# ben-hayes/neural-waveshaping-synthesis

Measured on AMD Instinct MI355X. Metric: audio_samples_per_sec, higher is better.
Workload: dtype f32 (fp16x2-split MFMA contractions = 22-bit products, fp32 accumulate; FiLM interpolation bf16x3-split MFMA = exact fp32 operands); 1 GPU; NEWT forward, vn checkpoint, FastNEWT LUT, batch 64/GPU x 500 frames (4 s @ 16 kHz), torch.rand F0/control, RNG draws on device; batch_per_gpu=64, frames=500, samples_per_utterance=64000, parallelism=batch-shard x1, exciter_opts=0, streams=2

## Files before the change

neural-waveshaping-synthesis_amd/build.py:

```python
import concurrent.futures as cf
import hashlib
import os
import subprocess
import sys

HERE = os.path.dirname(os.path.abspath(__file__))
CSRC = os.path.join(HERE, "csrc")
OBJ = os.path.join(HERE, "csrc", "_obj")
LIB = os.path.join(HERE, "libnws_hip.so")
OPS_LIB = os.path.join(HERE, "libnws_torch_ops.so")
PROBE_LIB = os.path.join(HERE, "libnws_probe.so")
SOURCES = ["exciter_newt.hip", "control_gru.hip", "frame_mlps.hip", "fir_noise.hip", "reverb_fft.hip", "forward.hip",
           "loudness.hip", "stages.hip", "generic.hip", "stream.hip", "queue_probe.hip", "exchange.hip"]
PROBE_SOURCES = ["coexec_probe.hip"]
FLAGS = ["--offload-arch=gfx950", "-O3", "-std=c++17", "-ffp-contract=off", "-fPIC", "-fvisibility=default",
         "-Wall", "-Wno-unused-function", "-Wno-pass-failed", "-Rpass-analysis=kernel-resource-usage"]
KEEP_SLP = ("fir_noise.hip", "control_gru.hip")
EXTRA_FLAGS = {src: ["-fno-slp-vectorize"] for src in SOURCES + PROBE_SOURCES if src not in KEEP_SLP}
FLAGS += [f for f in os.environ.get("NWS_EXTRA_HIPCC_FLAGS", "").split() if f]
LLVM_BIN = "/opt/rocm/lib/llvm/bin"
SWIZZLE_ALLOW = ("pk_probe_kernel", "pk_probe2_kernel", "pk_probe_mixed_kernel")


def _hipcc():
    for c in (os.environ.get("HIPCC"), "/opt/rocm/bin/hipcc", "hipcc"):
        if c and (os.path.isabs(c) and os.path.exists(c) or not os.path.isabs(c)):
            return c
    raise RuntimeError("hipcc not found")


def _stamp():
    h = hashlib.sha256((" ".join(FLAGS) + repr(sorted(EXTRA_FLAGS.items()))).encode())
    for f in sorted(os.listdir(CSRC)):
        p = os.path.join(CSRC, f)
        if os.path.isfile(p) and f != "torch_ops.cpp":
            h.update(f.encode())
            h.update(open(p, "rb").read())
    for hdr in ("nws_hip.h", "nws_hip_debug.h", "nws_probe.h"):
        h.update(open(os.path.join(HERE, "..", "include", hdr), "rb").read())
    return h.hexdigest()


def device_disassembly(obj):
    import tempfile
    with tempfile.TemporaryDirectory() as td:
        fat, co = os.path.join(td, "fat.bin"), os.path.join(td, "dev.co")
        r = subprocess.run([os.path.join(LLVM_BIN, "llvm-objcopy"), "--dump-section", f".hip_fatbin={fat}", obj,
                            os.path.join(td, "host.o")], capture_output=True, text=True)
        if r.returncode != 0:
            if "not found" in r.stderr:
                return ""
            raise RuntimeError(f"llvm-objcopy failed on {obj}: {r.stderr}")
        subprocess.run([os.path.join(LLVM_BIN, "clang-offload-bundler"), "--unbundle", "--type=o", f"--input={fat}",
                        "--targets=hipv4-amdgcn-amd-amdhsa--gfx950", f"--output={co}"], check=True, capture_output=True)
        return subprocess.run([os.path.join(LLVM_BIN, "llvm-objdump"), "-d", co], check=True, capture_output=True,
                              text=True).stdout


def check_packed_swizzles(obj, allow=None):
    import re
    allow = SWIZZLE_ALLOW if allow is None else allow
    found, kernel = [], None
    for line in device_disassembly(obj).splitlines():
        m = re.match(r"^[0-9a-f]+ <(\S+)>:", line)
        if m:
            kernel = m.group(1)
            continue
        m = re.search(r"\b(v_\w+)\b.*?op_sel:\[\d,(\d)", line)
        if m and m.group(2) == "1" and not any(a in (kernel or "") for a in allow):
            found.append((kernel, " ".join(line.split("//")[0].split())))
    return found


def _vgprs(tok):
    import re
    m = re.fullmatch(r"v\[(\d+):(\d+)\]", tok)
    if m:
        return set(range(int(m.group(1)), int(m.group(2)) + 1))
    m = re.fullmatch(r"v(\d+)", tok)
    return {int(m.group(1))} if m else set()


def check_valu_mfma_hazard(obj, wait_states=2):
    import re
    found, kernel, window = [], None, []
    for line in device_disassembly(obj).splitlines():
        m = re.match(r"^[0-9a-f]+ <(\S+)>:", line)
        if m:
            kernel, window = m.group(1), []
            continue
        parts = line.split("//")[0].split("\t")
        text = " ".join(" ".join(parts[1:]).split()) if len(parts) > 1 else ""
        if not text:
            continue
        op = text.split()[0]
        ops = [t.strip() for t in text[len(op):].split(",")]
        if op.startswith("v_mfma") or op.startswith("v_smfmac"):
            srcs = set().union(*[_vgprs(t.split()[0]) for t in ops[1:4] if t])
            left = wait_states
            for ws, dst, ptext in reversed(window):
                if left <= 0:
                    break
                if dst & srcs:
                    found.append((kernel, ptext, text))
                left -= ws
        if op == "s_nop":
            window.append((int(ops[0], 0) + 1, set(), text))
        elif op.startswith("s_cbranch") or op in ("s_branch", "s_barrier", "s_endpgm", "s_setpc_b64"):
            window = []
        elif op.startswith("v_") and not op.startswith("v_mfma") and not op.startswith("v_smfmac") and not op.startswith("v_cmp"):
            window.append((1, _vgprs(ops[0].split()[0]) if ops and ops[0] else set(), text))
        else:
            window.append((1, set(), text))
        window = window[-8:]
    return found


REGISTER_BUDGETS = (
    ("exciter_newt_kernelILi4ELi2ELi2E", 80, "default oscillator kernel: three 8-wave workgroups per CU"),
    ("exciter_newt_kernelILi4ELi2ELi6E", 80, "one-term variant: three 8-wave workgroups per CU"),
    ("exciter_newt_kernelILi4ELi2ELi10E", 80, "hybrid variant: three 8-wave workgroups per CU"),
    ("exciter_newt_kernelILi4ELi2ELi26E", 80, "hybrid-W variant: three 8-wave workgroups per CU"),
    ("exciter_newt_kernelILi5ELi1ELi0E", 128, "exact-shaper bank kernel: four 4-wave workgroups per CU (38.8 KB of LDS each)"),
    ("exciter_newt_kernelILi6ELi1ELi0E", 128, "exact-shaper bank kernel (no v_fract): four 4-wave workgroups per CU"),
    ("g_exciter_newt_mfma_kernel", 128, "runtime-size oscillator kernel: four 4-wave workgroups per CU"),
)


def kernel_registers(remarks):
    regs, name = {}, None
    for line in remarks.splitlines():
        if "Function Name:" in line:
            name = line.split("Function Name:")[1].split("[-Rpass")[0].strip()
            regs[name] = 0
        elif name is not None and (" VGPRs:" in line or " AGPRs:" in line) and "Spill" not in line:
            regs[name] += int(line.split("GPRs:")[1].split()[0])
    return regs


def check_register_budgets(remarks, budgets=None):
    over = []
    for kernel, n in kernel_registers(remarks).items():
        for key, budget, why in (REGISTER_BUDGETS if budgets is None else budgets):
            if key in kernel and n > budget:
                over.append((kernel, n, budget, why))
    return over


def build_torch_ops(force=False, verbose=True):
    try:
        import torch
        from torch.utils import cpp_extension as ce
    except Exception as e:
        print(f"torch not importable ({e}): skipping libnws_torch_ops.so", file=sys.stderr)
        return None
    src = os.path.join(CSRC, "torch_ops.cpp")
    h = hashlib.sha256(open(src, "rb").read())
    h.update(open(os.path.join(HERE, "..", "include", "nws_hip.h"), "rb").read())
    h.update(open(os.path.join(HERE, "..", "include", "nws_hip_debug.h"), "rb").read())
    h.update(torch.__version__.encode())
    stamp, stamp_file = h.hexdigest(), OPS_LIB + ".stamp"
    if not force and os.path.exists(OPS_LIB) and os.path.exists(stamp_file) and open(stamp_file).read() == stamp:
        return OPS_LIB
    tlib = os.path.join(os.path.dirname(torch.__file__), "lib")
    cmd = ["g++", "-O2", "-std=c++17", "-fPIC", "-shared", "-D__HIP_PLATFORM_AMD__", "-DUSE_ROCM",
           f"-D_GLIBCXX_USE_CXX11_ABI={int(torch._C._GLIBCXX_USE_CXX11_ABI)}", "-Wall", "-Wno-unused-function",
           *[f"-I{p}" for p in ce.include_paths()], "-I/opt/rocm/include", src, "-o", OPS_LIB,
           f"-L{HERE}", "-lnws_hip", f"-L{tlib}", "-ltorch", "-ltorch_cpu", "-lc10", "-lc10_hip", "-ltorch_hip",
           "-Wl,-rpath,$ORIGIN", f"-Wl,-rpath,{tlib}"]
    r = subprocess.run(cmd, capture_output=True, text=True)
    if r.returncode != 0:
        raise RuntimeError(f"g++ failed on torch_ops.cpp:\n{r.stderr[-6000:]}")
    with open(stamp_file, "w") as f:
        f.write(stamp)
    if verbose:
        print(f"built {OPS_LIB}")
    return OPS_LIB


def build(force=False, verbose=True):
    lib = build_hip(force, verbose)
    build_torch_ops(force, verbose)
    return lib


def build_hip(force=False, verbose=True):
    stamp_file = LIB + ".stamp"
    stamp = _stamp()
    if (not force and os.path.exists(LIB) and os.path.exists(PROBE_LIB) and os.path.exists(stamp_file)
            and open(stamp_file).read() == stamp):
        return LIB
    os.makedirs(OBJ, exist_ok=True)
    hipcc = _hipcc()

    def compile_one(src):
        obj = os.path.join(OBJ, src.replace(".hip", ".o"))
        cmd = [hipcc, *FLAGS, *EXTRA_FLAGS.get(src, []), "-c", os.path.join(CSRC, src), "-o", obj]
        r = subprocess.run(cmd, capture_output=True, text=True)
        if r.returncode != 0:
            raise RuntimeError(f"hipcc failed on {src}:\n{r.stderr}")
        name, spilled, rest, skip = None, [], [], 0
        for line in r.stderr.splitlines():
            if skip and (line.lstrip().startswith("|") or line.lstrip().split(" ")[0].isdigit()):
                skip -= 1
                continue
            skip = 0
            if "remark:" in line:
                skip = 2
                if "Function Name:" in line:
                    name = line.split("Function Name:")[1].split("[-Rpass")[0].strip()
                elif "ScratchSize [bytes/lane]:" in line and int(line.split("ScratchSize [bytes/lane]:")[1].split()[0]) != 0:
                    spilled.append(name)
            else:
                rest.append(line)
        if spilled:
            if os.environ.get("NWS_BUILD_ALLOW_SCRATCH") == "1":
                print(f"{src}: kernels using scratch memory (allowed by NWS_BUILD_ALLOW_SCRATCH): {spilled}", file=sys.stderr)
            else:
                raise RuntimeError(f"{src}: kernels using scratch memory (spills or stack): {spilled}")
        over = check_register_budgets(r.stderr)
        if over:
            lines = "\n".join(f"  {k}: {n} registers > {b} ({why})" for k, n, b, why in over)
            raise RuntimeError(f"{src}: kernels over their register budget (REGISTER_BUDGETS: workgroups per CU):\n{lines}")
        swz = check_packed_swizzles(obj, SWIZZLE_ALLOW if src in PROBE_SOURCES else ())
        if swz:
            lines = "\n".join(f"  {k}: {i}" for k, i in swz[:12])
            raise RuntimeError(f"{src}: packed fp32 instructions with a swizzled src1 low lane (co-execution hazard, see "
                               f"check_packed_swizzles):\n{lines}")
        haz = check_valu_mfma_hazard(obj)
        if haz:
            lines = "\n".join(f"  {k}: {p}  ->  {m}" for k, p, m in haz[:12])
            raise RuntimeError(f"{src}: v_mfma reads a VGPR that a VALU instruction wrote less than 2 wait states earlier (inline asm "
                               f"in front of a matrix instruction? see check_valu_mfma_hazard):\n{lines}")
        if verbose and "\n".join(rest).strip():
            print("\n".join(rest), file=sys.stderr)
        return obj

    with cf.ThreadPoolExecutor(max_workers=len(SOURCES) + len(PROBE_SOURCES)) as ex:
        objs = list(ex.map(compile_one, SOURCES + PROBE_SOURCES))
    for lib, these in ((LIB, objs[:len(SOURCES)]), (PROBE_LIB, objs[len(SOURCES):])):
        r = subprocess.run([hipcc, "--offload-arch=gfx950", "-shared", "-fPIC", *these, "-o", lib], capture_output=True, text=True)
        if r.returncode != 0:
            raise RuntimeError(f"link failed:\n{r.stderr}")
    with open(stamp_file, "w") as f:
        f.write(stamp)
    if verbose:
        print(f"built {LIB}")
    return LIB


if __name__ == "__main__":
    build(force="--force" in sys.argv)
```

neural-waveshaping-synthesis_amd/csrc/fir_noise.hip:

```cpp
#include <type_traits>

#include "nws_common.h"

namespace {

constexpr int kL = NWS_FIR_LEN;
constexpr int kHop = NWS_HOP;
constexpr int kHalf = NWS_FIR_HALF;
constexpr int kHopsPerBlock = 4;

struct NoiseLds {
  float taps[kHopsPerBlock + 1][kL];
  float taps1[kHopsPerBlock + 1][kL];
  float sig[(kHopsPerBlock + 1) * kHop + kHop];
};

__device__ __forceinline__ float padded_noise(const float* __restrict__ noise, int len, int origin, int i) {
  int s = i - origin;
  if (s < 0) s = -s;
  if (s > len - 1) s = 2 * (len - 1) - s;
  s = s < 0 ? 0 : s;
  return noise[s];
}

__device__ __forceinline__ float row_noise(const float* __restrict__ noise, int lo, int hi, int origin, int i) {
  int s = i - origin;
  if (s < lo) s = 2 * lo - s;
  if (s > hi) s = 2 * hi - s;
  s = s < 0 ? 0 : s;
  return noise[s];
}

template <bool ROWS>
__global__ __launch_bounds__(256) void fir_noise_kernel(const float* __restrict__ fir, const float* __restrict__ noise,
                                                        const float* __restrict__ add_in, int T, int len, int origin,
                                                        float* __restrict__ out, const int4* __restrict__ rows) {
  __shared__ __attribute__((aligned(16))) NoiseLds L;
  const int tid = threadIdx.x, lane = tid & 63, wave = tid >> 6;
  const int half = lane >> 5, q = lane & 31;
  const int b = blockIdx.y;
  const int t0 = blockIdx.x * kHopsPerBlock;
  const int N = T * kHop;
  int4 rb = make_int4(0, 0, 0, 0);
  if constexpr (ROWS) rb = rows[b];
  const int t_lo = ROWS ? rb.z : 0;

  for (int e = tid; e < (kHopsPerBlock + 1) * kL; e += 256) {
    const int fr = e >> 8, k = e & 255;
    const int t = t0 - 1 + fr;
    const int d = k >= kHalf ? k - kHalf : kHalf - k;
    const float v = (t >= t_lo && t < T && d < kHalf) ? fir[((size_t)b * T + t) * kHalf + d] : 0.0f;
    L.taps[fr][k] = v;
    L.taps1[fr][(k + 1) & 255] = v;
  }
  for (int e = tid; e < (kHopsPerBlock + 1) * kHop + kHop; e += 256) {
    const int i = (t0 - 1) * kHop + e;
    float v = 0.0f;
    if (i >= 0 && i < N + kL - 1) v = ROWS ? row_noise(noise, rb.x, rb.y, origin, i) : padded_noise(noise, len, origin, i);
    L.sig[e] = v;
  }
  __syncthreads();

  const int t = t0 + wave;
  if (t >= T) return;
  const int slot = wave + 1 - half;
  const int nb = half * kHop + 4 * q;
  const float* f = &L.sig[slot * kHop];
  const float* h = L.taps[slot];

  const float* h1 = L.taps1[slot];
  f32x2 a0 = {0.0f, 0.0f}, a1 = {0.0f, 0.0f}, a2 = {0.0f, 0.0f}, a3 = {0.0f, 0.0f};
  float4 hi0 = *reinterpret_cast<const float4*>(&h[nb & 255]);
  float4 hi1 = *reinterpret_cast<const float4*>(&h1[nb & 255]);
#pragma unroll 4
  for (int m0 = 0; m0 < kL; m0 += 4) {
    const float4 lo0 = *reinterpret_cast<const float4*>(&h[(nb - m0 - 4) & 255]);
    const float4 lo1 = *reinterpret_cast<const float4*>(&h1[(nb - m0 - 4) & 255]);
    const float4 fv = *reinterpret_cast<const float4*>(&f[m0]);
    const f32x2 fs0 = {fv.y, fv.x}, fs1 = {fv.w, fv.z};
    a1 = fma2(fs0, f32x2{hi0.x, hi0.y}, a1);
    a3 = fma2(fs0, f32x2{hi0.z, hi0.w}, a3);
    a1 = fma2(fs1, f32x2{lo0.z, lo0.w}, a1);
    a3 = fma2(fs1, f32x2{hi0.x, hi0.y}, a3);
    a0 = fma2(fs0, f32x2{hi1.x, hi1.y}, a0);
    a2 = fma2(fs0, f32x2{hi1.z, hi1.w}, a2);
    a0 = fma2(fs1, f32x2{lo1.z, lo1.w}, a0);
    a2 = fma2(fs1, f32x2{hi1.x, hi1.y}, a2);
    hi0 = lo0;
    hi1 = lo1;
  }
  const float y0 = a0.x + a0.y, y1 = a1.x + a1.y, y2 = a2.x + a2.y, y3 = a3.x + a3.y;
  const float o0 = y0 + nws_swap_halves(y0);
  const float o1 = y1 + nws_swap_halves(y1);
  const float o2 = y2 + nws_swap_halves(y2);
  const float o3 = y3 + nws_swap_halves(y3);
  if (half == 0) {
    const float inv = t == t_lo ? 1.0f : 0.5f;
    const size_t o = (size_t)b * N + (size_t)t * kHop + 4 * q;
    float4 r = make_float4(o0 * inv, o1 * inv, o2 * inv, o3 * inv);
    if (add_in != nullptr) {
      const float4 a = *reinterpret_cast<const float4*>(&add_in[o]);
      r.x = a.x + r.x;
      r.y = a.y + r.y;
      r.z = a.z + r.z;
      r.w = a.w + r.w;
    }
    *reinterpret_cast<float4*>(&out[o]) = r;
  }
}

constexpr int kUtt = 32;
constexpr int kCopyHalfs = 256;
constexpr unsigned kCopyRot = 0xD95D9510u;
__device__ __forceinline__ int copy_rot_halfs(int c) { return (int)((kCopyRot >> (4 * c)) & 15u) * 8; }
constexpr int kRowHalfs = 136;
constexpr float kNoiseScale = 1024.0f;
typedef _Float16 f16x8 __attribute__((ext_vector_type(8)));
typedef _Float16 f16x4 __attribute__((ext_vector_type(4)));

struct NoiseMfmaLds {
  _Float16 rhi[2][8][kCopyHalfs];
  _Float16 rlo[2][8][kCopyHalfs];
  _Float16 hhi[kUtt][kRowHalfs];
  _Float16 hlo[kUtt][kRowHalfs];
  __attribute__((aligned(16))) float unscale[kUtt];
  float win[4 * kHop];
};

typedef _Float16 f16x2 __attribute__((ext_vector_type(2)));

__device__ __forceinline__ void split16x2(float a, float b, f16x2& hi, f16x2& lo) {
  hi = __builtin_convertvector(f32x2{a, b}, f16x2);
  const unsigned hp = __builtin_bit_cast(unsigned, hi);
  unsigned lp;
  asm("v_fma_mixlo_f16 %0, %1, -1.0, %2 op_sel_hi:[1,0,0]" : "=v"(lp) : "v"(hp), "v"(a));
  asm("v_fma_mixhi_f16 %0, %1, -1.0, %2 op_sel:[1,0,0] op_sel_hi:[1,0,0]" : "+v"(lp) : "v"(hp), "v"(b));
  lo = __builtin_bit_cast(f16x2, lp);
}

template <int CTRL, int ROW_MASK>
__device__ __forceinline__ float dpp_f32(float v) {
  return __builtin_bit_cast(float, __builtin_amdgcn_update_dpp(0, __builtin_bit_cast(int, v), CTRL, ROW_MASK, 0xf, false));
}
__device__ __forceinline__ float half_max(float v) {
  v = fmaxf(v, dpp_f32<0xb1, 0xf>(v));
  v = fmaxf(v, dpp_f32<0x4e, 0xf>(v));
  v = fmaxf(v, dpp_f32<0x141, 0xf>(v));
  v = fmaxf(v, dpp_f32<0x140, 0xf>(v));
  const auto r = __builtin_amdgcn_permlane16_swap(__float_as_uint(v), __float_as_uint(v), false, false);
  return fmaxf(__uint_as_float(r[0]), __uint_as_float(r[1]));
}
__global__ __launch_bounds__(256, 4) void fir_noise_mfma_kernel(const float* __restrict__ fir, const float* __restrict__ noise,
                                                                const float* __restrict__ add_in, int B, int T, int len,
                                                                int origin, float* __restrict__ out) {
  __shared__ __attribute__((aligned(16))) NoiseMfmaLds L;
  const int tid = threadIdx.x, lane = tid & 63, wave = tid >> 6;
  const int kh = lane >> 5, col = lane & 31;
  const int per_xcd = gridDim.x >> 3;
  const int t = (blockIdx.x & 7) * per_xcd + (blockIdx.x >> 3);
  if (t >= T) return;
  const int b0 = blockIdx.y * kUtt;
  const int N = T * kHop;

  const int p32 = lane & 31;
  const int my_row = wave + 4 * kh;
  auto load_rows = [&](int frame, float4 (&v)[8]) {
#pragma unroll
    for (int it = 0; it < 4; ++it) {
      const int b = b0 + my_row + 8 * it;
      const bool ok = frame >= 0 && frame < T && b < B;
      const int bc = b < B ? b : B - 1, fc = frame < 0 ? 0 : (frame < T ? frame : T - 1);
      const float* src = &fir[((size_t)bc * T + fc) * kHalf + 4 * p32];
      const float* src_lo = &fir[((size_t)bc * T + fc) * kHalf + 4 * (31 - p32)];
      const float4 hi4 = *reinterpret_cast<const float4*>(src), lo4 = *reinterpret_cast<const float4*>(src_lo);
      const float4 zero4 = make_float4(0.0f, 0.0f, 0.0f, 0.0f);
      v[it + 4] = ok ? hi4 : zero4;
      v[it] = ok ? lo4 : zero4;
    }
  };
  float wv[2];
#pragma unroll
  for (int q = 0; q < 2; ++q) {
    const int e = tid + 256 * q, i = kHop * (t - 1) + e;
    const bool in = e < 3 * kHop && i >= 0 && i < N + kL - 1;
    const float nv = padded_noise(noise, len, origin, in ? i : origin);
    wv[q] = in ? nv * kNoiseScale : 0.0f;
  }
  float4 cur[8], prv[8];
  load_rows(t, cur);
  load_rows(t - 1, prv);
  L.win[tid] = wv[0];
  L.win[tid + 256] = wv[1];

  asm volatile("s_waitcnt lgkmcnt(0)\n\ts_barrier" ::: "memory");

#pragma unroll
  for (int fr = 0; fr < 2; ++fr) {
    const int c = tid & 7, v0 = 8 * (((tid >> 3) + (int)((0x25072500u >> (4 * c)) & 15u)) & 31);
    f16x8 h8, l8;
#pragma unroll
    for (int q = 0; q < 4; ++q) {
      const int u0 = (v0 + 2 * q + c) & 255, u1 = (v0 + 2 * q + 1 + c) & 255;
      const float a = fr == 0 ? L.win[kHop + ((-u0) & 255)] : L.win[(kHop - u0) & 255];
      const float bb = fr == 0 ? L.win[kHop + ((-u1) & 255)] : L.win[(kHop - u1) & 255];
      f16x2 hi, lo;
      split16x2(a, bb, hi, lo);
      h8[2 * q] = hi.x;
      h8[2 * q + 1] = hi.y;
      l8[2 * q] = lo.x;
      l8[2 * q + 1] = lo.y;
    }
    const int vp = (v0 + copy_rot_halfs(c)) & 255;
    *reinterpret_cast<f16x8*>(&L.rhi[fr][c][vp]) = h8;
    *reinterpret_cast<f16x8*>(&L.rlo[fr][c][vp]) = l8;
  }
  float scale[4];
#pragma unroll
  for (int it = 0; it < 4; ++it) {
    auto amax4 = [](const float4& a) { return fmaxf(fmaxf(fabsf(a.x), fabsf(a.y)), fmaxf(fabsf(a.z), fabsf(a.w))); };
    float mx = fmaxf(amax4(cur[it + 4]), amax4(prv[it + 4]));
    mx = half_max(mx);
    int ex = (int)((__float_as_uint(mx) >> 23) & 0xff);
    ex = ex < 16 ? 16 : (ex > 250 ? 250 : ex);
    scale[it] = __uint_as_float((unsigned)(268 - ex) << 23);
    if (p32 == 0) L.unscale[my_row + 8 * it] = __uint_as_float((unsigned)(ex - 14) << 23) * (1.0f / kNoiseScale);
  }
  auto stage_rows = [&](const float4 (&v)[8], const int khalf) {
#pragma unroll
    for (int it = 0; it < 4; ++it) {
      const int r = my_row + 8 * it;
      float4 t4 = v[it + 4 * khalf];
      if (khalf == 0) {
        float up = dpp_f32<0x138, 0xf>(t4.x);
        up = p32 == 0 ? 0.0f : up;
        t4 = make_float4(up, t4.w, t4.z, t4.y);
      }
      f16x2 h01, l01, h23, l23;
      split16x2(t4.x * scale[it], t4.y * scale[it], h01, l01);
      split16x2(t4.z * scale[it], t4.w * scale[it], h23, l23);
      const f16x4 h = {h01.x, h01.y, h23.x, h23.y}, l = {l01.x, l01.y, l23.x, l23.y};
      *reinterpret_cast<f16x4*>(&L.hhi[r][4 * p32]) = h;
      *reinterpret_cast<f16x4*>(&L.hlo[r][4 * p32]) = l;
    }
  };
  stage_rows(cur, 0);
  __syncthreads();

  f32x16 acc;
  const int j = 32 * wave + col;
  const int c = (-j) & 7;
  const int jr = j - copy_rot_halfs(c);
  auto accumulate = [&](const int fr, const int khalf, auto first_tag) {
    constexpr bool kFirst = decltype(first_tag)::value;
    const _Float16* rh = &L.rhi[fr][c][0];
    const _Float16* rl = &L.rlo[fr][c][0];
#pragma unroll 4
    for (int ks = 0; ks < kL / 32; ++ks) {
      const int k = 16 * ks + 8 * kh;
      const int s8 = ((kL / 2 * khalf + k - jr) & 255) & ~7;
      const f16x8 ahi = *reinterpret_cast<const f16x8*>(&L.hhi[col][k]);
      const f16x8 alo = *reinterpret_cast<const f16x8*>(&L.hlo[col][k]);
      const f16x8 bhi = *reinterpret_cast<const f16x8*>(&rh[s8]);
      const f16x8 blo = *reinterpret_cast<const f16x8*>(&rl[s8]);
      if (kFirst && ks == 0) acc = __builtin_amdgcn_mfma_f32_32x32x16_f16(ahi, bhi, f32x16{}, 0, 0, 0);
      else acc = __builtin_amdgcn_mfma_f32_32x32x16_f16(ahi, bhi, acc, 0, 0, 0);
      acc = __builtin_amdgcn_mfma_f32_32x32x16_f16(ahi, blo, acc, 0, 0, 0);
      acc = __builtin_amdgcn_mfma_f32_32x32x16_f16(alo, bhi, acc, 0, 0, 0);
    }
  };
  accumulate(0, 0, std::true_type{});
  __syncthreads();
  stage_rows(cur, 1);
  __syncthreads();
  accumulate(0, 1, std::false_type{});
  __syncthreads();
  stage_rows(prv, 0);
  __syncthreads();
  accumulate(1, 0, std::false_type{});
  __syncthreads();
  stage_rows(prv, 1);
  float addv[16];
  const bool has_add = add_in != nullptr;
#pragma unroll
  for (int r = 0; r < 16; ++r) {
    const int row = (r & 3) + 8 * (r >> 2) + 4 * kh;
    const int b = b0 + row < B ? b0 + row : B - 1;
    addv[r] = has_add ? add_in[(size_t)b * N + (size_t)t * kHop + j] : 0.0f;
  }
  __syncthreads();
  accumulate(1, 1, std::false_type{});

  const float ola = t == 0 ? 1.0f : 0.5f;
  float vout[16];
#pragma unroll
  for (int g = 0; g < 4; ++g) {
    const float4 us = *reinterpret_cast<const float4*>(&L.unscale[8 * g + 4 * kh]);
    const float u4[4] = {us.x, us.y, us.z, us.w};
#pragma unroll
    for (int i = 0; i < 4; ++i) {
      const float v = acc[4 * g + i] * (ola * u4[i]);
      vout[4 * g + i] = has_add ? addv[4 * g + i] + v : v;
    }
  }
  float* o = out + (size_t)(b0 + 4 * kh) * N + (size_t)t * kHop + j;
  if (b0 + kUtt <= B) {
#pragma unroll
    for (int r = 0; r < 16; ++r) o[(size_t)((r & 3) + 8 * (r >> 2)) * N] = vout[r];
  } else {
#pragma unroll
    for (int r = 0; r < 16; ++r) {
      const int row = (r & 3) + 8 * (r >> 2);
      if (b0 + 4 * kh + row < B) o[(size_t)row * N] = vout[r];
    }
  }
}

}

extern "C" int nws_fir_noise_window(const float* fir, const float* noise, int noise_len, int origin, const float* add_in,
                                    int B, int T, float* out, void* stream) {
  if (!fir || !noise || !out || B <= 0 || T <= 0 || noise_len < 2 || origin < 0) return NWS_ERR_BAD_ARG;
  if (B > 65535) return NWS_ERR_UNSUPPORTED;
  if (B >= 16) {
    const dim3 grid(8 * ((T + 7) / 8), (B + kUtt - 1) / kUtt);
    fir_noise_mfma_kernel<<<grid, 256, 0, (hipStream_t)stream>>>(fir, noise, add_in, B, T, noise_len, origin, out);
    NWS_CHECK_LAUNCH();
    return NWS_OK;
  }
  const dim3 grid((T + kHopsPerBlock - 1) / kHopsPerBlock, B);
  fir_noise_kernel<false><<<grid, 256, 0, (hipStream_t)stream>>>(fir, noise, add_in, T, noise_len, origin, out, nullptr);
  NWS_CHECK_LAUNCH();
  return NWS_OK;
}

extern "C" int nws_fir_noise_window_rows(const float* fir, const float* noise, int origin, const int4* rows, int B, int T,
                                         float* out, void* stream) {
  if (!fir || !noise || !out || !rows || B <= 0 || T <= 0 || origin < 0) return NWS_ERR_BAD_ARG;
  if (B > 65535) return NWS_ERR_UNSUPPORTED;
  const dim3 grid((T + kHopsPerBlock - 1) / kHopsPerBlock, B);
  fir_noise_kernel<true><<<grid, 256, 0, (hipStream_t)stream>>>(fir, noise, nullptr, T, 0, origin, out, rows);
  NWS_CHECK_LAUNCH();
  return NWS_OK;
}

extern "C" int nws_fir_noise(const float* fir, const float* noise, const float* add_in, int B, int T, float* out,
                             void* stream) {
  return nws_fir_noise_window(fir, noise, T * kHop - 1, kL / 2, add_in, B, T, out, stream);
}
```

Measured before the change: 10.41 billion samples/s.

## Replace MFMA FIR noise convolution with FFT-based spectral filtering kernel

Swaps the fp16-split MFMA direct convolution for windowed noise filtering with a 256-point FFT approach. The noise segments and FIR magnitude spectra are transformed per wave, multiplied in the frequency domain, inverse-transformed and overlap-added in registers. The kernel packs two utterances per lane with f32x2 vector math, and SLP vectorisation is turned off for the file. It aims to cut the O(L²) MAC count and the split-precision MFMA passes, at the cost of FFT shuffles, LDS transposes and different rounding behaviour.

```diff
diff --git a/neural-waveshaping-synthesis_amd/build.py b/neural-waveshaping-synthesis_amd/build.py
--- a/neural-waveshaping-synthesis_amd/build.py
+++ b/neural-waveshaping-synthesis_amd/build.py
@@ -15,7 +15,7 @@
 PROBE_SOURCES = ["coexec_probe.hip"]
 FLAGS = ["--offload-arch=gfx950", "-O3", "-std=c++17", "-ffp-contract=off", "-fPIC", "-fvisibility=default",
          "-Wall", "-Wno-unused-function", "-Wno-pass-failed", "-Rpass-analysis=kernel-resource-usage"]
-KEEP_SLP = ("fir_noise.hip", "control_gru.hip")
+KEEP_SLP = ("control_gru.hip",)
 EXTRA_FLAGS = {src: ["-fno-slp-vectorize"] for src in SOURCES + PROBE_SOURCES if src not in KEEP_SLP}
 FLAGS += [f for f in os.environ.get("NWS_EXTRA_HIPCC_FLAGS", "").split() if f]
 LLVM_BIN = "/opt/rocm/lib/llvm/bin"
diff --git a/neural-waveshaping-synthesis_amd/csrc/fir_noise.hip b/neural-waveshaping-synthesis_amd/csrc/fir_noise.hip
--- a/neural-waveshaping-synthesis_amd/csrc/fir_noise.hip
+++ b/neural-waveshaping-synthesis_amd/csrc/fir_noise.hip
@@ -1,6 +1,12 @@
-#include <type_traits>
-
 #include "nws_common.h"
+#include "fir_spectral_fft.h"
+
+template <>
+struct SpOps<f32x2> {
+  static __device__ __forceinline__ f32x2 fma(f32x2 a, f32x2 b, f32x2 c) { return __builtin_elementwise_fma(a, b, c); }
+  static __device__ __forceinline__ f32x2 of(float v) { return f32x2{v, v}; }
+  static __device__ __forceinline__ f32x2 at(const float* p) { return *reinterpret_cast<const f32x2*>(p); }
+};
 
 namespace {
 
@@ -109,208 +115,198 @@
   }
 }
 
-constexpr int kUtt = 32;
-constexpr int kCopyHalfs = 256;
-constexpr unsigned kCopyRot = 0xD95D9510u;
-__device__ __forceinline__ int copy_rot_halfs(int c) { return (int)((kCopyRot >> (4 * c)) & 15u) * 8; }
-constexpr int kRowHalfs = 136;
-constexpr float kNoiseScale = 1024.0f;
-typedef _Float16 f16x8 __attribute__((ext_vector_type(8)));
-typedef _Float16 f16x4 __attribute__((ext_vector_type(4)));
-
-struct NoiseMfmaLds {
-  _Float16 rhi[2][8][kCopyHalfs];
-  _Float16 rlo[2][8][kCopyHalfs];
-  _Float16 hhi[kUtt][kRowHalfs];
-  _Float16 hlo[kUtt][kRowHalfs];
-  __attribute__((aligned(16))) float unscale[kUtt];
-  float win[4 * kHop];
+constexpr int kSpWaves = 4;
+constexpr int kSpUtt = 2 * kSpWaves;
+constexpr int kSpPairs = 4;
+constexpr int kSpHops = 2 * kSpPairs - 1;
+
+struct SpectralLds {
+  float4 sd[kSpPairs][9][16];
+  float4 tw[256];
+  f32x2 x[kSpWaves][kSpPairs * kSpPlane];
 };
 
-typedef _Float16 f16x2 __attribute__((ext_vector_type(2)));
-
-__device__ __forceinline__ void split16x2(float a, float b, f16x2& hi, f16x2& lo) {
-  hi = __builtin_convertvector(f32x2{a, b}, f16x2);
-  const unsigned hp = __builtin_bit_cast(unsigned, hi);
-  unsigned lp;
-  asm("v_fma_mixlo_f16 %0, %1, -1.0, %2 op_sel_hi:[1,0,0]" : "=v"(lp) : "v"(hp), "v"(a));
-  asm("v_fma_mixhi_f16 %0, %1, -1.0, %2 op_sel:[1,0,0] op_sel_hi:[1,0,0]" : "+v"(lp) : "v"(hp), "v"(b));
-  lo = __builtin_bit_cast(f16x2, lp);
-}
-
-template <int CTRL, int ROW_MASK>
-__device__ __forceinline__ float dpp_f32(float v) {
-  return __builtin_bit_cast(float, __builtin_amdgcn_update_dpp(0, __builtin_bit_cast(int, v), CTRL, ROW_MASK, 0xf, false));
-}
-__device__ __forceinline__ float half_max(float v) {
-  v = fmaxf(v, dpp_f32<0xb1, 0xf>(v));
-  v = fmaxf(v, dpp_f32<0x4e, 0xf>(v));
-  v = fmaxf(v, dpp_f32<0x141, 0xf>(v));
-  v = fmaxf(v, dpp_f32<0x140, 0xf>(v));
-  const auto r = __builtin_amdgcn_permlane16_swap(__float_as_uint(v), __float_as_uint(v), false, false);
-  return fmaxf(__uint_as_float(r[0]), __uint_as_float(r[1]));
-}
-__global__ __launch_bounds__(256, 4) void fir_noise_mfma_kernel(const float* __restrict__ fir, const float* __restrict__ noise,
-                                                                const float* __restrict__ add_in, int B, int T, int len,
-                                                                int origin, float* __restrict__ out) {
-  __shared__ __attribute__((aligned(16))) NoiseMfmaLds L;
+__device__ __forceinline__ void sp_wave_sync() {
+  __builtin_amdgcn_fence(__ATOMIC_RELEASE, "wavefront");
+  __builtin_amdgcn_wave_barrier();
+  __builtin_amdgcn_fence(__ATOMIC_ACQUIRE, "wavefront");
+}
+
+template <class T>
+__device__ __forceinline__ void sp_transpose(T (&v)[16], T* x, int l) {
+#pragma unroll
+  for (int k = 0; k < 16; ++k) x[k * kSpRow + l] = v[k];
+  sp_wave_sync();
+#pragma unroll
+  for (int j = 0; j < 16; ++j) v[j] = x[l * kSpRow + j];
+  sp_wave_sync();
+}
+template <bool INV, class T>
+__device__ __forceinline__ void sp_fft256(C16T<T>& z, const float* tw, T* x, int l) {
+  sp_pass1<INV>(z, tw);
+  sp_transpose(z.re, x, l);
+  sp_transpose(z.im, x, l);
+  sp_dft16<INV>(z);
+}
+
+__device__ __forceinline__ f32x2 sp_shfl(f32x2 v, int src) { return f32x2{__shfl(v.x, src, 64), __shfl(v.y, src, 64)}; }
+__device__ __forceinline__ f32x2 sp_select(bool c, f32x2 a, f32x2 b) { return f32x2{c ? a.x : b.x, c ? a.y : b.y}; }
+
+__device__ __forceinline__ void sp_filter_spectrum(C16T<f32x2>& z, const f32x2 (&ua)[8], const f32x2 (&ub)[8], const float* tw,
+                                                   f32x2* x, int lane, int l) {
+  const int src = (lane & 48) | ((16 - l) & 15);
+  const f32x2 zero = {0.0f, 0.0f};
+#pragma unroll
+  for (int j = 0; j < 8; ++j) {
+    z.re[j] = ua[j];
+    z.im[j] = ub[j];
+  }
+#pragma unroll
+  for (int j = 8; j < 16; ++j) {
+    const f32x2 ma = sp_shfl(ua[15 - j], src), mb = sp_shfl(ub[15 - j], src);
+    const f32x2 oa = j == 8 ? zero : ua[(16 - j) & 7], ob = j == 8 ? zero : ub[(16 - j) & 7];
+    z.re[j] = sp_select(l == 0, oa, ma);
+    z.im[j] = sp_select(l == 0, ob, mb);
+  }
+  sp_fft256<false>(z, tw, x, l);
+}
+
+__global__ __launch_bounds__(64 * kSpWaves, 3) void fir_noise_spectral_kernel(const float* __restrict__ fir,
+                                                                             const float* __restrict__ noise,
+                                                                             const float* __restrict__ add_in, int B, int T, int len,
+                                                                             int origin, float* __restrict__ out, int nruns, int total) {
+  __shared__ __attribute__((aligned(16))) SpectralLds L;
   const int tid = threadIdx.x, lane = tid & 63, wave = tid >> 6;
-  const int kh = lane >> 5, col = lane & 31;
+  const int g = lane >> 4, l = lane & 15;
   const int per_xcd = gridDim.x >> 3;
-  const int t = (blockIdx.x & 7) * per_xcd + (blockIdx.x >> 3);
-  if (t >= T) return;
-  const int b0 = blockIdx.y * kUtt;
+  const int id = (blockIdx.x & 7) * per_xcd + (blockIdx.x >> 3);
+  if (id >= total) return;
+  const int run = id % nruns;
+  const int b0 = (id / nruns) * kSpUtt + 2 * wave, b1 = b0 + 1;
+  const int t0 = run * kSpHops;
+  const int ta = t0 - 1 + 2 * g, tb = ta + 1;
   const int N = T * kHop;
-
-  const int p32 = lane & 31;
-  const int my_row = wave + 4 * kh;
-  auto load_rows = [&](int frame, float4 (&v)[8]) {
-#pragma unroll
-    for (int it = 0; it < 4; ++it) {
-      const int b = b0 + my_row + 8 * it;
-      const bool ok = frame >= 0 && frame < T && b < B;
-      const int bc = b < B ? b : B - 1, fc = frame < 0 ? 0 : (frame < T ? frame : T - 1);
-      const float* src = &fir[((size_t)bc * T + fc) * kHalf + 4 * p32];
-      const float* src_lo = &fir[((size_t)bc * T + fc) * kHalf + 4 * (31 - p32)];
-      const float4 hi4 = *reinterpret_cast<const float4*>(src), lo4 = *reinterpret_cast<const float4*>(src_lo);
-      const float4 zero4 = make_float4(0.0f, 0.0f, 0.0f, 0.0f);
-      v[it + 4] = ok ? hi4 : zero4;
-      v[it] = ok ? lo4 : zero4;
-    }
-  };
-  float wv[2];
-#pragma unroll
-  for (int q = 0; q < 2; ++q) {
-    const int e = tid + 256 * q, i = kHop * (t - 1) + e;
-    const bool in = e < 3 * kHop && i >= 0 && i < N + kL - 1;
-    const float nv = padded_noise(noise, len, origin, in ? i : origin);
-    wv[q] = in ? nv * kNoiseScale : 0.0f;
-  }
-  float4 cur[8], prv[8];
-  load_rows(t, cur);
-  load_rows(t - 1, prv);
-  L.win[tid] = wv[0];
-  L.win[tid + 256] = wv[1];
-
-  asm volatile("s_waitcnt lgkmcnt(0)\n\ts_barrier" ::: "memory");
-
-#pragma unroll
-  for (int fr = 0; fr < 2; ++fr) {
-    const int c = tid & 7, v0 = 8 * (((tid >> 3) + (int)((0x25072500u >> (4 * c)) & 15u)) & 31);
-    f16x8 h8, l8;
-#pragma unroll
-    for (int q = 0; q < 4; ++q) {
-      const int u0 = (v0 + 2 * q + c) & 255, u1 = (v0 + 2 * q + 1 + c) & 255;
-      const float a = fr == 0 ? L.win[kHop + ((-u0) & 255)] : L.win[(kHop - u0) & 255];
-      const float bb = fr == 0 ? L.win[kHop + ((-u1) & 255)] : L.win[(kHop - u1) & 255];
-      f16x2 hi, lo;
-      split16x2(a, bb, hi, lo);
-      h8[2 * q] = hi.x;
-      h8[2 * q + 1] = hi.y;
-      l8[2 * q] = lo.x;
-      l8[2 * q + 1] = lo.y;
-    }
-    const int vp = (v0 + copy_rot_halfs(c)) & 255;
-    *reinterpret_cast<f16x8*>(&L.rhi[fr][c][vp]) = h8;
-    *reinterpret_cast<f16x8*>(&L.rlo[fr][c][vp]) = l8;
-  }
-  float scale[4];
-#pragma unroll
-  for (int it = 0; it < 4; ++it) {
-    auto amax4 = [](const float4& a) { return fmaxf(fmaxf(fabsf(a.x), fabsf(a.y)), fmaxf(fabsf(a.z), fabsf(a.w))); };
-    float mx = fmaxf(amax4(cur[it + 4]), amax4(prv[it + 4]));
-    mx = half_max(mx);
-    int ex = (int)((__float_as_uint(mx) >> 23) & 0xff);
-    ex = ex < 16 ? 16 : (ex > 250 ? 250 : ex);
-    scale[it] = __uint_as_float((unsigned)(268 - ex) << 23);
-    if (p32 == 0) L.unscale[my_row + 8 * it] = __uint_as_float((unsigned)(ex - 14) << 23) * (1.0f / kNoiseScale);
-  }
-  auto stage_rows = [&](const float4 (&v)[8], const int khalf) {
-#pragma unroll
-    for (int it = 0; it < 4; ++it) {
-      const int r = my_row + 8 * it;
-      float4 t4 = v[it + 4 * khalf];
-      if (khalf == 0) {
-        float up = dpp_f32<0x138, 0xf>(t4.x);
-        up = p32 == 0 ? 0.0f : up;
-        t4 = make_float4(up, t4.w, t4.z, t4.y);
-      }
-      f16x2 h01, l01, h23, l23;
-      split16x2(t4.x * scale[it], t4.y * scale[it], h01, l01);
-      split16x2(t4.z * scale[it], t4.w * scale[it], h23, l23);
-      const f16x4 h = {h01.x, h01.y, h23.x, h23.y}, l = {l01.x, l01.y, l23.x, l23.y};
-      *reinterpret_cast<f16x4*>(&L.hhi[r][4 * p32]) = h;
-      *reinterpret_cast<f16x4*>(&L.hlo[r][4 * p32]) = l;
-    }
-  };
-  stage_rows(cur, 0);
+  const bool oka = ta >= 0 && ta < T, okb = tb < T;
+  const int tac = ta < 0 ? 0 : (ta < T ? ta : T - 1), tbc = tb < T ? tb : T - 1;
+
+  const int bc0 = b0 < B ? b0 : B - 1, bc1 = b1 < B ? b1 : B - 1;
+  const float* rowa0 = &fir[((size_t)bc0 * T + tac) * kHalf + l];
+  const float* rowb0 = &fir[((size_t)bc0 * T + tbc) * kHalf + l];
+  const float* rowa1 = &fir[((size_t)bc1 * T + tac) * kHalf + l];
+  const float* rowb1 = &fir[((size_t)bc1 * T + tbc) * kHalf + l];
+  f32x2 ua[8], ub[8];
+#pragma unroll
+  for (int j = 0; j < 8; ++j) {
+    ua[j] = f32x2{rowa0[16 * j], rowa1[16 * j]};
+    ub[j] = f32x2{rowb0[16 * j], rowb1[16 * j]};
+  }
+  {
+    float c, s;
+    sp_twiddle((tid & 15) * (tid >> 4), c, s);
+    L.tw[tid] = make_float4(c, c, s, s);
+  }
+  const float* tw = reinterpret_cast<const float*>(&L.tw[l]);
   __syncthreads();
 
-  f32x16 acc;
-  const int j = 32 * wave + col;
-  const int c = (-j) & 7;
-  const int jr = j - copy_rot_halfs(c);
-  auto accumulate = [&](const int fr, const int khalf, auto first_tag) {
-    constexpr bool kFirst = decltype(first_tag)::value;
-    const _Float16* rh = &L.rhi[fr][c][0];
-    const _Float16* rl = &L.rlo[fr][c][0];
-#pragma unroll 4
-    for (int ks = 0; ks < kL / 32; ++ks) {
-      const int k = 16 * ks + 8 * kh;
-      const int s8 = ((kL / 2 * khalf + k - jr) & 255) & ~7;
-      const f16x8 ahi = *reinterpret_cast<const f16x8*>(&L.hhi[col][k]);
-      const f16x8 alo = *reinterpret_cast<const f16x8*>(&L.hlo[col][k]);
-      const f16x8 bhi = *reinterpret_cast<const f16x8*>(&rh[s8]);
-      const f16x8 blo = *reinterpret_cast<const f16x8*>(&rl[s8]);
-      if (kFirst && ks == 0) acc = __builtin_amdgcn_mfma_f32_32x32x16_f16(ahi, bhi, f32x16{}, 0, 0, 0);
-      else acc = __builtin_amdgcn_mfma_f32_32x32x16_f16(ahi, bhi, acc, 0, 0, 0);
-      acc = __builtin_amdgcn_mfma_f32_32x32x16_f16(ahi, blo, acc, 0, 0, 0);
-      acc = __builtin_amdgcn_mfma_f32_32x32x16_f16(alo, bhi, acc, 0, 0, 0);
-    }
-  };
-  accumulate(0, 0, std::true_type{});
+  f32x2* x = &L.x[wave][g * kSpPlane];
+  if (wave == 0) {
+    C16 z;
+    float* xs = reinterpret_cast<float*>(x);
+#pragma unroll
+    for (int j = 0; j < 16; ++j) {
+      const int i0 = kHop * ta + 16 * j + l, i1 = i0 + kHop;
+      const bool in0 = i0 >= 0 && i0 < N + kL - 1, in1 = i1 >= 0 && i1 < N + kL - 1;
+      const float v0 = padded_noise(noise, len, origin, in0 ? i0 : origin);
+      const float v1 = padded_noise(noise, len, origin, in1 ? i1 : origin);
+      z.re[j] = in0 ? v0 : 0.0f;
+      z.im[j] = in1 ? v1 : 0.0f;
+    }
+    sp_fft256<false>(z, tw, xs, l);
+    float mr[16], mi[16];
+    auto mirror = [&](const float (&v)[16], float (&m)[16]) {
+#pragma unroll
+      for (int j = 0; j < 16; ++j) xs[l + 16 * j] = v[j];
+      sp_wave_sync();
+#pragma unroll
+      for (int j = 0; j < 16; ++j) m[j] = xs[(256 - (l + 16 * j)) & 255];
+      sp_wave_sync();
+    };
+    mirror(z.re, mr);
+    mirror(z.im, mi);
+    const float c = (l & 1) ? -(1.0f / 512.0f) : (1.0f / 512.0f);
+#pragma unroll
+    for (int j = 0; j < 9; ++j)
+      L.sd[g][j][l] = make_float4(c * (z.re[j] + mr[j]), c * (z.im[j] - mi[j]), c * (z.re[j] - mr[j]), c * (z.im[j] + mi[j]));
+  }
+  const f32x2 zero = {0.0f, 0.0f};
+#pragma unroll
+  for (int j = 0; j < 8; ++j) {
+    ua[j] = sp_select(oka, ua[j], zero);
+    ub[j] = sp_select(okb, ub[j], zero);
+  }
+  C16T<f32x2> z;
+  sp_filter_spectrum(z, ua, ub, tw, x, lane, l);
   __syncthreads();
-  stage_rows(cur, 1);
-  __syncthreads();
-  accumulate(0, 1, std::false_type{});
-  __syncthreads();
-  stage_rows(prv, 0);
-  __syncthreads();
-  accumulate(1, 0, std::false_type{});
-  __syncthreads();
-  stage_rows(prv, 1);
-  float addv[16];
+
   const bool has_add = add_in != nullptr;
-#pragma unroll
-  for (int r = 0; r < 16; ++r) {
-    const int row = (r & 3) + 8 * (r >> 2) + 4 * kh;
-    const int b = b0 + row < B ? b0 + row : B - 1;
-    addv[r] = has_add ? add_in[(size_t)b * N + (size_t)t * kHop + j] : 0.0f;
-  }
-  __syncthreads();
-  accumulate(1, 1, std::false_type{});
-
-  const float ola = t == 0 ? 1.0f : 0.5f;
-  float vout[16];
-#pragma unroll
-  for (int g = 0; g < 4; ++g) {
-    const float4 us = *reinterpret_cast<const float4*>(&L.unscale[8 * g + 4 * kh]);
-    const float u4[4] = {us.x, us.y, us.z, us.w};
-#pragma unroll
-    for (int i = 0; i < 4; ++i) {
-      const float v = acc[4 * g + i] * (ola * u4[i]);
-      vout[4 * g + i] = has_add ? addv[4 * g + i] + v : v;
-    }
-  }
-  float* o = out + (size_t)(b0 + 4 * kh) * N + (size_t)t * kHop + j;
-  if (b0 + kUtt <= B) {
-#pragma unroll
-    for (int r = 0; r < 16; ++r) o[(size_t)((r & 3) + 8 * (r >> 2)) * N] = vout[r];
-  } else {
-#pragma unroll
-    for (int r = 0; r < 16; ++r) {
-      const int row = (r & 3) + 8 * (r >> 2);
-      if (b0 + 4 * kh + row < B) o[(size_t)row * N] = vout[r];
+  const bool sta = g > 0 && ta < T, stb = tb < T;
+  const size_t oa0 = (size_t)bc0 * N + (size_t)tac * kHop + l, ob0 = (size_t)bc0 * N + (size_t)tbc * kHop + l;
+  const size_t oa1 = (size_t)bc1 * N + (size_t)tac * kHop + l, ob1 = (size_t)bc1 * N + (size_t)tbc * kHop + l;
+  f32x2 adda[8], addb[8];
+  if (has_add) {
+#pragma unroll
+    for (int j = 0; j < 8; ++j) {
+      adda[j] = f32x2{add_in[oa0 + 16 * j], add_in[oa1 + 16 * j]};
+      addb[j] = f32x2{add_in[ob0 + 16 * j], add_in[ob1 + 16 * j]};
+    }
+  }
+  const float4* sdm = &L.sd[g][l == 0 ? 1 : 0][(16 - l) & 15];
+#pragma unroll
+  for (int j = 0; j < 16; ++j) {
+    const f32x2 ga = z.re[j], gb = z.im[j];
+    if (j < 9) {
+      const float4 sd = L.sd[g][j][l];
+      z.re[j] = f32x2{fmaf(ga.x, sd.x, gb.x * sd.z), fmaf(ga.y, sd.x, gb.y * sd.z)};
+      z.im[j] = f32x2{fmaf(ga.x, sd.y, gb.x * sd.w), fmaf(ga.y, sd.y, gb.y * sd.w)};
+    } else {
+      const float4 sd = sdm[(15 - j) * 16];
+      z.re[j] = f32x2{fmaf(ga.x, sd.x, -(gb.x * sd.z)), fmaf(ga.y, sd.x, -(gb.y * sd.z))};
+      z.im[j] = f32x2{fmaf(gb.x, sd.w, -(ga.x * sd.y)), fmaf(gb.y, sd.w, -(ga.y * sd.y))};
+    }
+  }
+  sp_fft256<true>(z, tw, x, l);
+  const float invb = tb == 0 ? 1.0f : 0.5f;
+  f32x2 ha[8], hb[8];
+#pragma unroll
+  for (int j = 0; j < 8; ++j) {
+    const f32x2 ya0 = sp_select(oka, z.re[j], zero), ya1 = sp_select(oka, z.re[j + 8], zero);
+    const f32x2 yb0 = sp_select(okb, z.im[j], zero), yb1 = sp_select(okb, z.im[j + 8], zero);
+    const f32x2 prev = sp_shfl(yb1, (lane - 16) & 63);
+    ha[j] = (ya0 + prev) * 0.5f;
+    hb[j] = (yb0 + ya1) * invb;
+    if (has_add) {
+      ha[j] = adda[j] + ha[j];
+      hb[j] = addb[j] + hb[j];
+    }
+  }
+  if (sta) {
+    if (b0 < B) {
+#pragma unroll
+      for (int j = 0; j < 8; ++j) out[oa0 + 16 * j] = ha[j].x;
+    }
+    if (b1 < B) {
+#pragma unroll
+      for (int j = 0; j < 8; ++j) out[oa1 + 16 * j] = ha[j].y;
+    }
+  }
+  if (stb) {
+    if (b0 < B) {
+#pragma unroll
+      for (int j = 0; j < 8; ++j) out[ob0 + 16 * j] = hb[j].x;
+    }
+    if (b1 < B) {
+#pragma unroll
+      for (int j = 0; j < 8; ++j) out[ob1 + 16 * j] = hb[j].y;
     }
   }
 }
@@ -322,8 +318,11 @@
   if (!fir || !noise || !out || B <= 0 || T <= 0 || noise_len < 2 || origin < 0) return NWS_ERR_BAD_ARG;
   if (B > 65535) return NWS_ERR_UNSUPPORTED;
   if (B >= 16) {
-    const dim3 grid(8 * ((T + 7) / 8), (B + kUtt - 1) / kUtt);
-    fir_noise_mfma_kernel<<<grid, 256, 0, (hipStream_t)stream>>>(fir, noise, add_in, B, T, noise_len, origin, out);
+    const long long nruns = (T + kSpHops - 1) / kSpHops, total = nruns * ((B + kSpUtt - 1) / kSpUtt);
+    if (total > (1ll << 30)) return NWS_ERR_UNSUPPORTED;
+    const dim3 grid((unsigned)(8 * ((total + 7) / 8)));
+    fir_noise_spectral_kernel<<<grid, 64 * kSpWaves, 0, (hipStream_t)stream>>>(fir, noise, add_in, B, T, noise_len, origin, out,
+                                                                             (int)nruns, (int)total);
     NWS_CHECK_LAUNCH();
     return NWS_OK;
   }
diff --git a/neural-waveshaping-synthesis_amd/csrc/fir_spectral_fft.h b/neural-waveshaping-synthesis_amd/csrc/fir_spectral_fft.h
--- /dev/null
+++ b/neural-waveshaping-synthesis_amd/csrc/fir_spectral_fft.h
@@ -0,0 +1,112 @@
+#pragma once
+
+#ifndef NWS_SP_FN
+#define NWS_SP_FN __device__ __forceinline__
+#endif
+#ifndef NWS_SP_TABLE
+#define NWS_SP_TABLE __device__ const
+#endif
+
+template <class T>
+struct C16T {
+  T re[16], im[16];
+};
+typedef C16T<float> C16;
+
+template <class T>
+struct SpOps {
+  static NWS_SP_FN T fma(T a, T b, T c) { return fmaf(a, b, c); }
+  static NWS_SP_FN T of(float v) { return v; }
+  static NWS_SP_FN T at(const float* p) { return p[0]; }
+};
+
+NWS_SP_TABLE float kSpCosQ[65] = {
+    1.0f, 0.999698818f, 0.99879545f, 0.997290432f, 0.99518472f, 0.992479563f, 0.989176512f, 0.985277653f, 0.980785251f,
+    0.975702107f, 0.970031261f, 0.963776052f, 0.956940353f, 0.949528158f, 0.941544056f, 0.932992816f, 0.923879504f,
+    0.914209783f, 0.903989315f, 0.893224299f, 0.881921291f, 0.870086968f, 0.857728601f, 0.84485358f, 0.831469595f,
+    0.817584813f, 0.803207517f, 0.78834641f, 0.773010433f, 0.757208824f, 0.740951121f, 0.724247098f, 0.707106769f,
+    0.689540565f, 0.671558976f, 0.653172851f, 0.634393275f, 0.615231574f, 0.59569931f, 0.575808167f, 0.555570245f,
+    0.534997642f, 0.514102757f, 0.492898196f, 0.471396744f, 0.449611336f, 0.427555084f, 0.405241311f, 0.382683426f,
+    0.359895051f, 0.336889863f, 0.313681751f, 0.290284663f, 0.266712755f, 0.242980182f, 0.219101235f, 0.195090324f,
+    0.170961887f, 0.146730468f, 0.122410677f, 0.0980171412f, 0.0735645667f, 0.0490676761f, 0.024541229f, 0.0f};
+
+NWS_SP_FN void sp_twiddle(int m, float& c, float& s) {
+  const int q = m >> 6, r = m & 63;
+  const float a = kSpCosQ[r], b = kSpCosQ[64 - r];
+  c = q == 0 ? a : (q == 1 ? -b : (q == 2 ? -a : b));
+  s = q == 0 ? b : (q == 1 ? a : (q == 2 ? -b : -a));
+}
+
+template <bool INV, class T>
+NWS_SP_FN void sp_cmul(T& re, T& im, T cc, T s) {
+  const T sg = INV ? -s : s;
+  const T r = SpOps<T>::fma(re, cc, im * sg), i = SpOps<T>::fma(im, cc, -(re * sg));
+  re = r;
+  im = i;
+}
+
+template <bool INV, class T>
+NWS_SP_FN void sp_dft4(T& r0, T& i0, T& r1, T& i1, T& r2, T& i2, T& r3, T& i3) {
+  const T sr0 = r0 + r2, si0 = i0 + i2, dr0 = r0 - r2, di0 = i0 - i2;
+  const T sr1 = r1 + r3, si1 = i1 + i3, dr1 = r1 - r3, di1 = i1 - i3;
+  if (!INV) {
+    r1 = dr0 + di1; i1 = di0 - dr1;
+    r3 = dr0 - di1; i3 = di0 + dr1;
+  } else {
+    r1 = dr0 - di1; i1 = di0 + dr1;
+    r3 = dr0 + di1; i3 = di0 - dr1;
+  }
+  r0 = sr0 + sr1; i0 = si0 + si1;
+  r2 = sr0 - sr1; i2 = si0 - si1;
+}
+
+template <bool INV, class T>
+NWS_SP_FN void sp_dft16(C16T<T>& v) {
+  constexpr float kC[10] = {1.0f, 0.92387953251128674f, 0.70710678118654752f, 0.38268343236508977f, 0.0f,
+                            -0.38268343236508977f, -0.70710678118654752f, -0.92387953251128674f, -1.0f, -0.92387953251128674f};
+  constexpr float kS[10] = {0.0f, 0.38268343236508977f, 0.70710678118654752f, 0.92387953251128674f, 1.0f,
+                            0.92387953251128674f, 0.70710678118654752f, 0.38268343236508977f, 0.0f, -0.38268343236508977f};
+#pragma unroll
+  for (int n2 = 0; n2 < 4; ++n2)
+    sp_dft4<INV>(v.re[n2], v.im[n2], v.re[4 + n2], v.im[4 + n2], v.re[8 + n2], v.im[8 + n2], v.re[12 + n2], v.im[12 + n2]);
+#pragma unroll
+  for (int k1 = 1; k1 < 4; ++k1) {
+#pragma unroll
+    for (int n2 = 1; n2 < 4; ++n2) {
+      const int m = n2 * k1, e = 4 * k1 + n2;
+      if (m == 4) {
+        const T r = INV ? -v.im[e] : v.im[e], i = INV ? v.re[e] : -v.re[e];
+        v.re[e] = r;
+        v.im[e] = i;
+      } else {
+        sp_cmul<INV>(v.re[e], v.im[e], SpOps<T>::of(kC[m]), SpOps<T>::of(kS[m]));
+      }
+    }
+  }
+#pragma unroll
+  for (int k1 = 0; k1 < 4; ++k1)
+    sp_dft4<INV>(v.re[4 * k1], v.im[4 * k1], v.re[4 * k1 + 1], v.im[4 * k1 + 1], v.re[4 * k1 + 2], v.im[4 * k1 + 2],
+                 v.re[4 * k1 + 3], v.im[4 * k1 + 3]);
+#pragma unroll
+  for (int a = 0; a < 4; ++a) {
+#pragma unroll
+    for (int b = a + 1; b < 4; ++b) {
+      const T r = v.re[4 * a + b], i = v.im[4 * a + b];
+      v.re[4 * a + b] = v.re[4 * b + a];
+      v.im[4 * a + b] = v.im[4 * b + a];
+      v.re[4 * b + a] = r;
+      v.im[4 * b + a] = i;
+    }
+  }
+}
+
+constexpr int kSpRow = 17;
+constexpr int kSpPlane = 16 * kSpRow;
+constexpr int kSpTwStride = 64;
+
+template <bool INV, class T>
+NWS_SP_FN void sp_pass1(C16T<T>& z, const float* tw) {
+  sp_dft16<INV>(z);
+#pragma unroll
+  for (int k = 1; k < 16; ++k) sp_cmul<INV>(z.re[k], z.im[k], SpOps<T>::at(&tw[kSpTwStride * k]), SpOps<T>::at(&tw[kSpTwStride * k + 2]));
+}
```

Result: faster. 10.56 billion samples/s (median of 6 runs) (+1.4%).
